# csiro-robotics/ohm

Hardware: AMD Instinct MI355X
Metric: rays/sec integrated (occupancy) (higher is better)
Workload: dtype f64

## Files before the change

### include/ohmhip.h

```cpp
#ifndef OHMHIP_H
#define OHMHIP_H

#include <stddef.h>
#include <stdint.h>

#ifdef __cplusplus
extern "C" {
#endif

#define OHMHIP_EXPERIMENTAL

#define OHMHIP_OK 0
#define OHMHIP_ERR_INVALID_ARG (-1)
#define OHMHIP_ERR_NO_DEVICE (-2)
#define OHMHIP_ERR_CAPACITY (-3)
#define OHMHIP_ERR_UNSUPPORTED (-4)
#define OHMHIP_ERR_NOT_FOUND (-5)
#define OHMHIP_ERR_INTERNAL (-6)
#define OHMHIP_ERR_PEER (-7)

const char *ohmhip_error_string(int status);
const char *ohmhip_build_id(void);

typedef struct ohmhip_stream_s *ohmhip_stream_t;
// ... 152 lines not shown
                                     const float *d_intensities, const double *d_timestamps, unsigned ray_flags,
                                     size_t *integrated);
typedef struct ohmhip_cache_stats
{
  uint64_t hits;
  uint64_t misses;
  uint64_t full;
  uint32_t regions_resident;
  uint32_t region_capacity;
  uint64_t bytes_per_region;
  uint64_t memory_limit;
  uint64_t evictions;
  uint64_t readmissions;
  uint32_t regions_spilled;
  uint32_t spill_enabled;
  uint64_t writebacks;
  uint64_t writeback_hits;
  uint64_t writeback_stale;
} ohmhip_cache_stats;
int ohmhip_map_cache_stats(ohmhip_map_t map, ohmhip_cache_stats *stats, int reset);
int ohmhip_map_set_memory_limit(ohmhip_map_t map, uint64_t bytes);
int ohmhip_map_set_spill_to_host(ohmhip_map_t map, int enable);
OHMHIP_EXPERIMENTAL int ohmhip_map_set_spill_writeback(ohmhip_map_t map, int enable);
int ohmhip_map_sync(ohmhip_map_t map);
int ohmhip_map_last_stats(ohmhip_map_t map, ohmhip_batch_stats *stats);

OHMHIP_EXPERIMENTAL int ohmhip_map_batch_timings(ohmhip_map_t map, uint32_t batches_back, float ms[4]);
OHMHIP_EXPERIMENTAL int ohmhip_map_set_phase_timing(ohmhip_map_t map, int enable);
OHMHIP_EXPERIMENTAL int ohmhip_map_reserve_rays(ohmhip_map_t map, size_t ray_count);
int ohmhip_map_set_first_ray_time(ohmhip_map_t map, double time);
int ohmhip_map_first_ray_time(ohmhip_map_t map, double *time);
OHMHIP_EXPERIMENTAL int ohmhip_map_batches_launched(ohmhip_map_t map, uint64_t *count);
OHMHIP_EXPERIMENTAL int ohmhip_map_pipeline_counts(ohmhip_map_t map, uint64_t *batches, uint64_t *binned_early);
OHMHIP_EXPERIMENTAL int ohmhip_map_rays_beyond_tiles(ohmhip_map_t map, uint64_t *count);

int ohmhip_map_region_count(ohmhip_map_t map, size_t *count);
int ohmhip_map_regions(ohmhip_map_t map, int16_t *keys_xyz, size_t capacity, size_t *count);
int ohmhip_map_dirty_regions(ohmhip_map_t map, int16_t *keys_xyz, size_t capacity, size_t *count);
int ohmhip_map_clear_dirty(ohmhip_map_t map);
size_t ohmhip_layer_voxel_bytes(int layer_id);

int ohmhip_map_read_regions(ohmhip_map_t map, int layer_id, const int16_t *keys_xyz, size_t count, void *const *dsts);
int ohmhip_map_write_regions(ohmhip_map_t map, int layer_id, const int16_t *keys_xyz, size_t count,
                             const void *const *srcs);
int ohmhip_map_clear(ohmhip_map_t map);
int ohmhip_map_remove_regions(ohmhip_map_t map, const int16_t *keys_xyz, size_t count, size_t *removed);

int ohmhip_map_line_keys(ohmhip_map_t map, const double *lines, size_t line_count, uint32_t max_keys_per_line,
                         void *keys_out, uint32_t *counts_out);

int ohmhip_map_rays_query(ohmhip_map_t map, const double *rays, size_t element_count, double volume_coefficient,
                          double *ranges, double *unobserved_volumes, int8_t *terminal_types, void *terminal_keys);
OHMHIP_EXPERIMENTAL int ohmhip_map_rays_query_device(ohmhip_map_t map, const double *d_rays, size_t element_count,
                                                     double volume_coefficient, double *d_ranges,
                                                     double *d_unobserved_volumes, int8_t *d_terminal_types,
                                                     void *d_terminal_keys);

#define OHMHIP_QF_UNKNOWN_AS_OCCUPIED (1u << 0)
#define OHMHIP_QF_REPORT_UNSCALED (1u << 4)
typedef struct ohmhip_clearance_params
{
  float search_radius;
  float axis_scaling[3];
  unsigned flags;
} ohmhip_clearance_params;

// ... 264 lines not shown
```

### ohm_amd/_lib.py

```python
import ctypes as C
import os

_HERE = os.path.dirname(os.path.abspath(__file__))
LIB_PATH = os.environ.get("OHMHIP_LIB") or os.path.join(_HERE, "lib", "libohmhip.so")


class OhmHipError(RuntimeError):
    def __init__(self, status, what=""):
        self.status = status
        msg = lib.ohmhip_error_string(status).decode() if "lib" in globals() else str(status)
        super().__init__(f"{what}: [{status}] {msg}" if what else f"[{status}] {msg}")


if not os.path.exists(LIB_PATH):
    raise ImportError(
        f"{LIB_PATH} is missing: build it with `python -c 'import __graft_entry__ as g; g.build()'` "
        "(hipcc --offload-arch=gfx950). ohm_amd has no CPU fallback.")

lib = C.CDLL(LIB_PATH)

OK = 0
ERR_INVALID_ARG, ERR_NO_DEVICE, ERR_CAPACITY, ERR_UNSUPPORTED, ERR_NOT_FOUND, ERR_INTERNAL, ERR_PEER = (-1, -2, -3, -4,
                                                                                                       -5, -6, -7)
MERGE_SHARED_ONLY, MERGE_FULL_UNION = 0, 1
# ... 172 lines not shown
    "ohmhip_map_sync": (C.c_int, [_vp]),
    "ohmhip_map_last_stats": (C.c_int, [_vp, C.POINTER(BatchStats)]),
    "ohmhip_map_region_count": (C.c_int, [_vp, C.POINTER(C.c_size_t)]),
    "ohmhip_map_regions": (C.c_int, [_vp, _vp, C.c_size_t, C.POINTER(C.c_size_t)]),
    "ohmhip_map_dirty_regions": (C.c_int, [_vp, _vp, C.c_size_t, C.POINTER(C.c_size_t)]),
    "ohmhip_map_clear_dirty": (C.c_int, [_vp]),
    "ohmhip_map_read_regions": (C.c_int, [_vp, C.c_int, _vp, C.c_size_t, _vp]),
    "ohmhip_map_write_regions": (C.c_int, [_vp, C.c_int, _vp, C.c_size_t, _vp]),
    "ohmhip_map_clear": (C.c_int, [_vp]),
    "ohmhip_map_remove_regions": (C.c_int, [_vp, _vp, C.c_size_t, C.POINTER(C.c_size_t)]),
    "ohmhip_transform_samples": (C.c_int, [_vp, _vp, _vp, C.c_uint32, _vp, _vp, C.c_uint32, C.c_double, _vp, _vp,
                                           C.POINTER(C.c_uint32)]),
    "ohmhip_pattern_create": (C.c_int, [_vp, C.c_size_t, C.POINTER(_vp)]),
    "ohmhip_pattern_destroy": (C.c_int, [_vp]),
    "ohmhip_pattern_ray_count": (C.c_int, [_vp, C.POINTER(C.c_size_t)]),
    "ohmhip_pattern_build_rays": (C.c_int, [_vp, _vp, C.c_size_t, C.c_int, C.c_double, _vp]),
    "ohmhip_pattern_last_rays": (C.c_int, [_vp, _vp, C.POINTER(C.c_size_t)]),
    "ohmhip_map_apply_pattern": (C.c_int, [_vp, _vp, _vp, C.c_size_t, C.c_int, C.c_double, C.c_float, C.c_uint,
                                           C.POINTER(C.c_size_t)]),
    "ohmhip_map_can_copy": (C.c_int, [_vp, _vp]),
    "ohmhip_map_copy": (C.c_int, [_vp, _vp, C.POINTER(CopyParams), C.POINTER(CopyStats)]),
    "ohmhip_map_compare": (C.c_int, [_vp, _vp, C.POINTER(CompareParams), C.c_uint64, _vp, C.c_uint64, _vp,
                                     C.POINTER(CompareResult)]),
    "ohmhip_map_compare_device": (C.c_int, [_vp, _vp, C.POINTER(CompareParams), C.c_uint64, _vp, C.c_uint64, _vp, _vp]),
    "ohmhip_map_batch_timings": (C.c_int, [_vp, C.c_uint32, C.POINTER(C.c_float)]),
    "ohmhip_comm_exchange_side": (C.c_int, [_vp, _vp, _vp, _vp, _vp, C.c_uint32, _vp]),
    "ohmhip_gather_rows": (C.c_int, [_vp, _vp, C.c_size_t, C.c_uint32, _vp, _vp]),
    "ohmhip_map_reserve_rays": (C.c_int, [_vp, C.c_size_t]),
    "ohmhip_map_set_first_ray_time": (C.c_int, [_vp, C.c_double]),
    "ohmhip_map_first_ray_time": (C.c_int, [_vp, C.POINTER(C.c_double)]),
    "ohmhip_map_set_phase_timing": (C.c_int, [_vp, C.c_int]),
    "ohmhip_map_batches_launched": (C.c_int, [_vp, C.POINTER(C.c_uint64)]),
    "ohmhip_map_pipeline_counts": (C.c_int, [_vp, C.POINTER(C.c_uint64), C.POINTER(C.c_uint64)]),
    "ohmhip_map_rays_beyond_tiles": (C.c_int, [_vp, C.POINTER(C.c_uint64)]),
    "ohmhip_map_line_keys": (C.c_int, [_vp, _vp, C.c_size_t, C.c_uint32, _vp, _vp]),
    "ohmhip_map_rays_query": (C.c_int, [_vp, _vp, C.c_size_t, C.c_double, _vp, _vp, _vp, _vp]),
    "ohmhip_map_rays_query_device": (C.c_int, [_vp, _vp, C.c_size_t, C.c_double, _vp, _vp, _vp, _vp]),
    "ohmhip_map_clearance_regions": (C.c_int, [_vp, _vp, C.c_size_t, _vp, _vp]),
    "ohmhip_map_clearance_regions_device": (C.c_int, [_vp, _vp, C.c_size_t, _vp, _vp]),
    "ohmhip_map_clearance_keys": (C.c_int, [_vp, _vp, C.c_size_t, _vp, _vp]),
    "ohmhip_map_clearance_stale_regions": (C.c_int, [_vp, _vp, _vp, C.c_size_t, C.POINTER(C.c_size_t)]),
    "ohmhip_map_clearance_update": (C.c_int, [_vp, _vp, C.c_size_t, C.POINTER(C.c_size_t), C.POINTER(C.c_size_t)]),
    "ohmhip_map_clearance_update_regions": (C.c_int, [_vp, _vp, C.c_size_t, _vp, C.c_int, C.POINTER(C.c_size_t)]),
    "ohmhip_map_heightmap_extents": (C.c_int, [_vp, C.POINTER(HeightmapParams), C.POINTER(HeightmapExtents)]),
    "ohmhip_map_heightmap": (C.c_int, [_vp, C.POINTER(HeightmapParams), _vp, _vp, _vp, _vp, C.POINTER(C.c_uint64),
                                       C.POINTER(C.c_uint64)]),
    "ohmhip_map_heightmap_device": (C.c_int, [_vp, C.POINTER(HeightmapParams), _vp, _vp, _vp, _vp, _vp]),
    "ohmhip_map_heightmap_fill_extents": (C.c_int, [_vp, C.POINTER(HeightmapParams), C.POINTER(HeightmapExtents)]),
    "ohmhip_map_heightmap_fill": (C.c_int, [_vp, C.POINTER(HeightmapParams), _vp, _vp, _vp, _vp, _vp, C.c_uint64,
                                            C.POINTER(HeightmapFillStats)]),
    "ohmhip_map_heightmap_fill_device": (C.c_int, [_vp, C.POINTER(HeightmapParams), _vp, _vp, _vp, _vp, _vp, C.c_uint64,
                                                   C.POINTER(HeightmapFillStats)]),
    "ohmhip_map_cloud_count": (C.c_int, [_vp, C.POINTER(CloudParams), C.POINTER(C.c_uint64)]),
    "ohmhip_map_cloud": (C.c_int, [_vp, C.POINTER(CloudParams), C.c_uint64, _vp, _vp, _vp, C.POINTER(C.c_uint64)]),
    "ohmhip_map_cloud_device": (C.c_int, [_vp, C.POINTER(CloudParams), C.c_uint64, _vp, _vp, _vp, _vp]),
    "ohmhip_map_nearest_neighbours": (C.c_int, [_vp, _vp, C.c_size_t, C.POINTER(NeighboursParams), C.c_uint64, _vp, _vp,
                                                _vp, C.POINTER(C.c_uint64)]),
    "ohmhip_map_nearest_neighbours_device": (C.c_int, [_vp, _vp, C.c_size_t, C.POINTER(NeighboursParams), C.c_uint64,
                                                       _vp, _vp, _vp, _vp]),
    "ohmhip_map_voxel_keys": (C.c_int, [_vp, _vp, C.c_size_t, _vp]),
    "ohmhip_map_read_voxels": (C.c_int, [_vp, C.c_int, _vp, C.c_size_t, _vp, _vp]),
    "ohmhip_map_read_voxels_device": (C.c_int, [_vp, C.c_int, _vp, C.c_size_t, _vp, _vp]),
    "ohmhip_map_filter_points": (C.c_int, [_vp, _vp, C.c_uint64, C.POINTER(PointFilterParams), C.c_uint64, _vp, _vp, _vp,
                                           _vp, C.POINTER(C.c_uint64)]),
    "ohmhip_map_filter_points_device": (C.c_int, [_vp, _vp, C.c_uint64, C.c_uint64, C.POINTER(PointFilterParams),
                                                  C.c_uint64, _vp, _vp, _vp, _vp, _vp]),
# ... 46 lines not shown
```

### ohm_amd/csrc/batch_run.h

```cpp
#ifndef OHMHIP_BATCH_RUN_H
#define OHMHIP_BATCH_RUN_H

namespace
{
struct BatchRun
{
  ohmhip_map_t m;
  const double *d_rays;
  const float *d_intensities;
  const double *d_timestamps;
  uint32_t n_rays;
  unsigned ray_flags;
  hipStream_t s, f;
  const Event *tev;
  uint32_t ring;
  uint32_t next_info_index = 0;
  bool info_clean = false;
  uint32_t ray_blocks = 0, bin_rays_per_block = 0, bin_threads = 0, bin_blocks = 0, bin_tab_mask = 0;
  uint32_t batch_chunk_segments = 0;
  int mode = 0;
  bool stop_mode = false, occupancy_mode = false, ndt_mode = false, tsdf_mode = false;
  bool occ_inline = false;
  int ray_shift = 0;
  SecondaryLayers sec;
// ... 73 lines not shown
    }
    if (occupancy_mode)
    {
      OHMHIP_CHECK(m->hit_keys_a.ensure(sizeof(unsigned long long) * size_t(n_rays), false, s));
      OHMHIP_CHECK(m->hit_keys_b.ensure(sizeof(unsigned long long) * size_t(n_rays), false, s));
      OHMHIP_CHECK(m->interval_counts.ensure(sizeof(uint32_t) * size_t(n_rays), true, s));
      size_t sort_bytes = 0;
      OHMHIP_CHECK(rocprim::radix_sort_keys<SortConfig>(nullptr, sort_bytes, static_cast<unsigned long long *>(m->hit_keys_a.ptr),
                                            static_cast<unsigned long long *>(m->hit_keys_b.ptr), size_t(n_rays),
                                            kHitRayBits, sortEndBit(m), s));
      OHMHIP_CHECK(m->sort_temp.ensure(sort_bytes, false, s));
    }
    return OHMHIP_OK;
  }

  uint32_t *binMask() const { return occupancy_mode ? nullptr : m->pool.d_hit_mask.get(); }

  void launchBin(bool bucket, uint32_t seg_capacity, unsigned long long *hit_keys, hipStream_t stream)
  {
    const auto pow2 = [](int v) { return (v & (v - 1)) == 0; };
    const bool plain = m->mc.owner_world <= 1u && pow2(m->mc.dim[0]) && pow2(m->mc.dim[1]) && pow2(m->mc.dim[2]);
    const bool small = bin_tab_mask < kLtabSmall;
    const auto kernel = small ? (plain ? k_ray_bin<kLtabSmall, true> : k_ray_bin<kLtabSmall, false>) :
                                (plain ? k_ray_bin<kLtabSize, true> : k_ray_bin<kLtabSize, false>);
    hipExtLaunchKernelGGL(kernel, dim3(bin_blocks), dim3(bin_threads), 0, stream, nullptr, tev[1], 0, m->mc,
                          regionTable(m), batchScratch(m), static_cast<const RayWalk *>(batchWalks(m).ptr), n_rays,
                          static_cast<Segment *>(m->segments.ptr), seg_capacity, hit_keys, binMask(), ray_shift,
                          bucket ? 1 : 0, bin_rays_per_block, bin_tab_mask);
    mark(1);
    m->tev_pre_walk[ring] = 1;
    m->bin_done_event = tev[1];
  }

  void launchRegionSort(uint32_t dense)
  {
    const unsigned long long *in = static_cast<const unsigned long long *>(m->hit_keys_a.ptr);
    unsigned long long *out = static_cast<unsigned long long *>(m->hit_keys_b.ptr);
    const bool need_dense = kSortSmallHits == 0 || dense > kSortSmallHits;
    if (need_dense)
    {
      hipExtLaunchKernelGGL((k_sort_region_hits<kSortRegionHits, kSortThreads>), dim3(2 * m->walk_workgroups),
                            dim3(kSortThreads), 0, s, nullptr, kSortSmallHits ? nullptr : tev[2].handle, 0, regionTable(m),
                            batchScratch(m), in, out, m->mc.region_voxels, kSortSmallHits, m->pool.d_hit_mask.get());
    }
    if (kSortSmallHits)
    {
      hipExtLaunchKernelGGL((k_sort_region_hits<kSortSmallHits ? kSortSmallHits : 64u, kSortSmallThreads>),
                            dim3(8 * m->walk_workgroups), dim3(kSortSmallThreads), 0, s, nullptr, tev[2], 0,
                            regionTable(m), batchScratch(m), in, out, m->mc.region_voxels, 0u, m->pool.d_hit_mask.get());
    }
    sort_covers = need_dense ? kSortRegionHits : kSortSmallHits;
    mark(2);
    m->tev_pre_walk[ring] = 2;
  }

  void launchDenseSort()
  {
    hipExtLaunchKernelGGL((k_sort_region_hits<kSortRegionHits, kSortThreads>), dim3(2 * m->walk_workgroups),
                          dim3(kSortThreads), 0, s, nullptr, tev[2], 0, regionTable(m), batchScratch(m),
                          static_cast<const unsigned long long *>(m->hit_keys_a.ptr),
                          static_cast<unsigned long long *>(m->hit_keys_b.ptr), m->mc.region_voxels, kSortSmallHits,
                          m->pool.d_hit_mask.get());
    sort_covers = kSortRegionHits;
  }

  int frontHalf()
  {
    if (m->batch_done_event[m->parity])
    {
      OHMHIP_CHECK(hipStreamWaitEvent(f, m->batch_done_event[m->parity], 0));
    }
    if (m->bin_done_event)
    {
      OHMHIP_CHECK(hipStreamWaitEvent(f, m->bin_done_event, 0));
    }
    if (attempt > 0 || !info_clean)
    {
      OHMHIP_CHECK(hipMemsetAsync(m->d_info + m->info_index, 0, sizeof(BatchInfo), f));
    }
    if (m->phase_timing)
    {
      OHMHIP_CHECK(hipEventRecord(tev[0], f));
      mark(0);
    }
    if (bin_tab_mask < kLtabSmall)
    {
      hipLaunchKernelGGL(k_ray_setup<kLtabSmall>, dim3(bin_blocks), dim3(bin_threads), 0, f, m->mc, regionTable(m),
                         batchScratch(m), d_rays, n_rays, ray_flags, static_cast<RayWalk *>(batchWalks(m).ptr),
                         bin_rays_per_block, bin_tab_mask);
    }
    else
    {
      hipLaunchKernelGGL(k_ray_setup<kLtabSize>, dim3(bin_blocks), dim3(bin_threads), 0, f, m->mc, regionTable(m),
                         batchScratch(m), d_rays, n_rays, ray_flags, static_cast<RayWalk *>(batchWalks(m).ptr),
                         bin_rays_per_block, bin_tab_mask);
// ... 623 lines not shown
```

### ohm_amd/csrc/map_state.h

```cpp
#ifndef OHMHIP_MAP_STATE_H
#define OHMHIP_MAP_STATE_H

namespace
{
const size_t kLayerBytes[OHMHIP_LID_COUNT] = { 4, 8, 24, 4, 4, 4, 8, 8, 8, 4 };

inline uint32_t layerClearWord(int l)
{
  return (l == OHMHIP_LID_OCCUPANCY) ? 0x7f800000u : (l == OHMHIP_LID_CLEARANCE) ? 0xbf800000u : 0u;
}


struct DevBuf
{
  void *ptr = nullptr;
  size_t bytes = 0;

  DevBuf() = default;
  DevBuf(DevBuf &&o) noexcept : ptr(o.ptr), bytes(o.bytes) { o.ptr = nullptr, o.bytes = 0; }
  DevBuf &operator=(DevBuf &&o) noexcept
  {
    if (this != &o)
    {
      release();
// ... 314 lines not shown
    DevBuf clear_regions, clear_keys, clear_out, clear_mask;
    DevBuf hm_winner, hm_rec_occ, hm_rec_vox, hm_rec_mean, hm_counts, hm_out_occ, hm_out_vox, hm_out_mean, hm_out_col;
    DevBuf hmf_grid, hmf_queue, hmf_ground, hmf_rec_cell, hmf_keys_a, hmf_keys_b, hmf_accept, hmf_accept_at, hmf_temp, hmf_log;
    PinnedBuf<uint32_t> hmf_next;
    DevBuf cloud_chunks, cloud_pos, cloud_keys, cloud_values;
    ScanScratch cloud_scan;
    DevBuf nn_chunks, nn_chunk_begin, nn_near, nn_best, nn_query_counts, nn_query_best, nn_keys, nn_ranges;
    ScanScratch nn_scan, nn_query_scan;
    DevBuf rv_keys, rv_values, rv_present;
    DevBuf pf_points, pf_status, pf_values, pf_keys, pf_kept;
    ScanScratch pf_scan;
    PinnedBuf<char> pf_staging;
    DevBuf compare_chunks, compare_records, compare_keys, compare_missing, compare_result;
    ScanScratch compare_scan;
  } query;
  struct ClearanceLayerState
  {
    struct Region
    {
      uint32_t changed = 0;
      uint32_t written = 0;
      uint32_t params = 0;
    };
    std::unordered_map<uint64_t, Region> regions;
    uint32_t epoch = 0;
    std::vector<ohmhip_clearance_params> param_sets;
    DevBuf table_keys, table_changed, present, written, stale;
  } clearance_layer;
  DevArray<uint32_t> d_event_count;
  uint32_t walk_workgroups = 256;
  bool walk_half = false;
  uint32_t walkSlots() const { return walk_workgroups * (walk_half ? 2u : 1u); }
  DevArray<unsigned long long> d_dbg;
  double first_ray_time = -1.0;
  uint32_t event_demand = 0;
  uint32_t event_limit = 0;
  bool spec_bucket_ok = false;
  uint32_t spec_max_region_hits = 0;
  double segments_per_ray = 10.0;
  uint32_t bin_rays_per_block = kBinRaysPerBlock;
  uint32_t min_chunk_segments = 2048;
  uint32_t chunk_segments = kChunkSegments;
  unsigned debug_flags = 0;
  int refill_min_idle = kRefillMinIdle;
  PinnedBuf<void> h_stage;
  size_t h_stage_bytes = 0;

  struct RaySlot
  {
    PinnedBuf<char> h;
    size_t capacity = 0;
    DevBuf d_rays, d_times, d_intens, d_fflags;
    Event uploaded;
    Event done;
    bool in_flight = false;
    bool rays_uploaded = false;
  } ray_slots[2];
  std::unique_ptr<StagePool> stage_pool;
  bool async_launch = false;
  std::unique_ptr<StagePool> launch_thread;
  bool launch_busy = false;
  int launch_result = OHMHIP_OK;
  int fill_slot = 0;
  size_t pending_rays = 0;
  size_t pending_calls = 0;
  unsigned pending_flags = 0;
// ... 124 lines not shown
```

### ohm_amd/csrc/ohmhip_map.hip

```cpp
#include <cstring>
#include <string.h>

#include "apply_kernels.h"
#include "batch_scratch.h"
#include "pool_kernels.h"
#include "ray_front_kernels.h"
#include "region_table.h"
#include "sample_sort_kernels.h"
#include "walk_kernel.h"
#include "replay_kernels.h"
#include "traversal_kernels.h"
#include "query_kernels.h"
#include "clearance_kernels.h"
#include "heightmap_kernels.h"
#include "heightmap_fill_kernels.h"
#include "cloud_kernels.h"
#include "neighbours_kernels.h"
#include "point_filter_kernels.h"
#include "copy_kernels.h"
#include "compare_kernels.h"

#include <rocprim/rocprim.hpp>

#include <algorithm>
// ... 139 lines not shown
    mc.fix_scale = double(kFixMaxDelta) / (1.01 * diagonal);
    mc.fix_margin = 2u * uint32_t(std::max(mc.dim[0], std::max(mc.dim[1], mc.dim[2]))) + 8u;
  }
  applyValueConfig(m);

  if (hipGetDevice(&m->device) != hipSuccess)
  {
    return OHMHIP_ERR_NO_DEVICE;
  }
  OHMHIP_CHECK(m->stream.create());
  OHMHIP_CHECK(m->copy_stream.create());
  OHMHIP_CHECK(m->front_stream.create());
  for (auto &e : m->ev)
  {
    OHMHIP_CHECK(e.create());
  }
  for (auto &set : m->tev)
  {
    for (auto &e : set)
    {
      OHMHIP_CHECK(e.create());
    }
  }
  for (auto &sl : m->ray_slots)
  {
    OHMHIP_CHECK(sl.uploaded.create(hipEventDisableTiming));
    OHMHIP_CHECK(sl.done.create(hipEventDisableTiming));
  }
  OHMHIP_CHECK(m->d_n_slots.alloc(sizeof(uint32_t)));
  OHMHIP_CHECK(m->d_info.alloc(3 * sizeof(BatchInfo)));
  OHMHIP_CHECK(m->d_event_count.alloc(8 * sizeof(uint32_t)));
  OHMHIP_CHECK(m->d_dbg.alloc(kDbgWords * sizeof(unsigned long long)));
  (void)hipMemset(m->d_dbg, 0, kDbgWords * sizeof(unsigned long long));
  OHMHIP_CHECK(m->h_info.alloc(2 * sizeof(BatchInfo), hipHostMallocMapped | hipHostMallocCoherent));
  std::memset(m->h_info, 0, 2 * sizeof(BatchInfo));
  OHMHIP_CHECK(m->h_passed.alloc(64, hipHostMallocMapped | hipHostMallocCoherent));
  OHMHIP_CHECK(m->ev_passed.create(hipEventDisableTiming));

  uint32_t capacity = m->config.region_capacity;
  if (capacity == 0)
  {
    const uint64_t budget = m->config.gpu_mem_size ? m->config.gpu_mem_size : (uint64_t(4) << 30);
    capacity = uint32_t(std::max<uint64_t>(64, budget / bytesPerRegionAllLayers(m->config, mc.region_voxels)));
  }
  capacity = std::min<uint32_t>(capacity, kMaxRegionSlots);
  OHMHIP_CHECK(allocPool(m, capacity, 0));
  {
    int device = 0, cus = 0;
    if (hipGetDevice(&device) == hipSuccess &&
        hipDeviceGetAttribute(&cus, hipDeviceAttributeMultiprocessorCount, device) == hipSuccess && cus > 0)
    {
      m->walk_workgroups = uint32_t(cus);
    }
  }
  if (const char *env = std::getenv("OHMHIP_CHUNK_SEGMENTS"))
  {
    m->chunk_segments = uint32_t(std::max(64, std::min(int(kMaxChunkSegments), std::atoi(env))));
  }
  if (const char *env = std::getenv("OHMHIP_EVENT_LIMIT"))
  {
    m->event_limit = uint32_t(std::max(0, std::atoi(env)));
  }
  if (const char *env = std::getenv("OHMHIP_WRITEBACK"))
  {
    m->writeback_off = std::atoi(env) == 0;
  }
  if (const char *env = std::getenv("OHMHIP_WRITEBACK_WGS"))
  {
    m->writeback_workgroups = uint32_t(std::max(1, std::min(4096, std::atoi(env))));
  }
  if (const char *env = std::getenv("OHMHIP_BIN_RAYS"))
  {
    m->bin_rays_per_block = uint32_t(std::max(128, std::min(int(kBinRaysPerBlock), std::atoi(env))));
  }
  if (const char *env = std::getenv("OHMHIP_MIN_CHUNK_SEGMENTS"))
  {
    m->min_chunk_segments = uint32_t(std::max(64, std::min(int(kMaxChunkSegments), std::atoi(env))));
  }
  if (const char *env = std::getenv("OHMHIP_EARLY_BIN"))
  {
    m->early_bin = std::atoi(env) != 0;
  }
  uint32_t half_voxels = uint32_t(WalkHalf::kTileVoxels) / 4u;
  if (const char *env = std::getenv("OHMHIP_WALK_HALF_VOXELS"))
  {
    half_voxels = uint32_t(std::max(0, std::min(int(WalkHalf::kTileVoxels), std::atoi(env))));
// ... 435 lines not shown
int ohmhip_map_batches_launched(ohmhip_map_t m, uint64_t *count)
try
{
  if (!m || !count)
  {
    return OHMHIP_ERR_INVALID_ARG;
  }
  if (m->launch_busy)
  {
    m->launch_thread->wait();
  }
  *count = m->batch_seq;
  return OHMHIP_OK;
}
OHMHIP_ABI_CATCH

int ohmhip_map_pipeline_counts(ohmhip_map_t m, uint64_t *batches, uint64_t *binned_early)
try
{
  if (!m || !batches || !binned_early)
  {
    return OHMHIP_ERR_INVALID_ARG;
  }
  if (m->launch_busy)
  {
    m->launch_thread->wait();
  }
  *batches = m->count_batches;
  *binned_early = m->count_binned_early;
  return OHMHIP_OK;
}
OHMHIP_ABI_CATCH

int ohmhip_map_cache_stats(ohmhip_map_t m, ohmhip_cache_stats *stats, int reset)
try
{
  if (!m || !stats)
  {
    return OHMHIP_ERR_INVALID_ARG;
  }
  OHMHIP_SETTLE(m);
  stats->hits = m->cache_hits;
  stats->misses = m->cache_misses;
  stats->full = m->cache_full;
  stats->regions_resident = m->slots_committed;
  stats->region_capacity = m->pool.slot_capacity;
  stats->bytes_per_region = bytesPerRegionAllLayers(m->config, m->mc.region_voxels);
  stats->memory_limit = m->memory_limit;
  stats->evictions = m->evictions;
  stats->readmissions = m->readmissions;
  stats->regions_spilled = uint32_t(m->spilled.size());
  stats->spill_enabled = m->spill_enabled ? 1u : 0u;
  stats->writebacks = m->writebacks;
  stats->writeback_hits = m->writeback_hits;
  stats->writeback_stale = m->writeback_stale;
  if (reset)
  {
    m->cache_hits = m->cache_misses = m->cache_full = 0;
    m->evictions = m->readmissions = 0;
    m->writebacks = m->writeback_hits = m->writeback_stale = 0;
  }
  return OHMHIP_OK;
}
OHMHIP_ABI_CATCH

int ohmhip_map_set_memory_limit(ohmhip_map_t m, uint64_t bytes)
// ... 198 lines not shown
```

### ohm_amd/csrc/sample_sort_kernels.h

```cpp
#ifndef OHMHIP_SAMPLE_SORT_KERNELS_H
#define OHMHIP_SAMPLE_SORT_KERNELS_H

#include "batch_scratch.h"
#include "region_table.h"

namespace ohmhip
{
__global__ void __launch_bounds__(256)
  k_hit_bounds(const unsigned long long *__restrict__ sorted, BatchScratch bs, int region_voxels,
               uint32_t *__restrict__ hit_mask)
{
  const uint32_t n_hits = bs.info->n_hits;
  const uint32_t i = blockIdx.x * blockDim.x + threadIdx.x;
  if (i >= n_hits)
  {
    return;
  }
  const unsigned long long group = hitGroup(sorted[i]);
  if (i == 0 || hitGroup(sorted[i - 1]) != group)
  {
    const uint32_t slot = hitSlot(sorted[i]);
    const uint32_t vi = hitVoxel(sorted[i]);
    bs.voxel_first_hit[size_t(slot) * size_t(region_voxels) + vi] = i;
    atomicOr(&hit_mask[size_t(slot) * (uint32_t(region_voxels + 31) >> 5) + (vi >> 5)], 1u << (vi & 31));
// ... 21 lines not shown
  const uint32_t low = g & ((1u << s_shift) - 1u);
  const uint32_t base = ((g >> s_shift) << (s_shift + R)) | low;
  const bool ascending = (base & k) == 0;
  unsigned long long v[kCount];
#pragma unroll
  for (uint32_t m = 0; m < kCount; ++m)
  {
    v[m] = l_keys[sortSlot(base | (m << s_shift))];
  }
#pragma unroll
  for (int t = 0; t < R; ++t)
  {
    const uint32_t d = 1u << (R - 1 - t);
#pragma unroll
    for (uint32_t m = 0; m < kCount; ++m)
    {
      if ((m & d) == 0)
      {
        const unsigned long long a = v[m];
        const unsigned long long c = v[m | d];
        const bool swap = (a > c) == ascending;
        v[m] = swap ? c : a;
        v[m | d] = swap ? a : c;
      }
    }
  }
#pragma unroll
  for (uint32_t m = 0; m < kCount; ++m)
  {
    l_keys[sortSlot(base | (m << s_shift))] = v[m];
  }
}

constexpr uint32_t kSortRegionHits = 8192;
constexpr int kSortThreads = 1024;
#ifndef OHMHIP_SORT_SMALL
#define OHMHIP_SORT_SMALL 2048
#endif
constexpr uint32_t kSortSmallHits = OHMHIP_SORT_SMALL;
constexpr int kSortSmallThreads = 256;

template <uint32_t kCap, int kThreads>
__global__ void __launch_bounds__(kThreads)
  k_sort_region_hits(RegionTable rt, BatchScratch bs, const unsigned long long *__restrict__ keys,
                     unsigned long long *__restrict__ sorted, int region_voxels, uint32_t min_hits,
                     uint32_t *__restrict__ hit_mask)
{
  __shared__ unsigned long long l_keys[kCap + kCap / 32];
  const uint32_t mask_words = uint32_t(region_voxels + 31) >> 5;
  const uint32_t n_regions = bs.info->n_hit_regions;
  for (uint32_t list_index = blockIdx.x; list_index < n_regions; list_index += gridDim.x)
  {
  const uint32_t h = bs.sort_list[list_index];
  const uint32_t slot = rt.vals[h];
  if (slot >= rt.slot_capacity)
  {
    continue;
  }
  const uint32_t begin = bs.hit_begin[slot];
  const uint32_t n = bs.hit_end[slot] - begin;
  if (n <= min_hits || n > kCap)
  {
    continue;
  }
  uint32_t padded = 64;
  while (padded < n)
  {
    padded <<= 1;
  }
  for (uint32_t i = threadIdx.x; i < padded; i += kThreads)
  {
    l_keys[sortSlot(i)] = (i < n) ? keys[begin + i] : ~0ull;
  }
  __syncthreads();
  for (uint32_t k = 2; k <= padded; k <<= 1)
  {
    uint32_t j = k >> 1;
    while (j > 0)
    {
      const uint32_t levels_left = uint32_t(32 - __clz(int(j)));
      const uint32_t r = min(3u, levels_left);
      const uint32_t s_shift = levels_left - r;
      const uint32_t group_count = padded >> r;
      for (uint32_t g = threadIdx.x; g < group_count; g += kThreads)
      {
        if (r == 3)
        {
          bitonicFused<3>(l_keys, g, s_shift, k);
        }
        else if (r == 2)
        {
          bitonicFused<2>(l_keys, g, s_shift, k);
        }
        else
        {
          bitonicFused<1>(l_keys, g, s_shift, k);
        }
      }
      __syncthreads();
      j >>= r;
    }
  }
  for (uint32_t base = 0; base < n; base += kThreads)
  {
    const uint32_t i = base + threadIdx.x;
    uint32_t word = 0xffffffffu, bits = 0;
    if (i < n)
    {
      const unsigned long long key = l_keys[sortSlot(i)];
      sorted[begin + i] = key;
      const uint32_t vi = hitVoxel(key);
      word = vi >> 5;
      if (i == 0 || hitGroup(l_keys[sortSlot(i - 1)]) != hitGroup(key))
      {
        bs.voxel_first_hit[size_t(slot) * size_t(region_voxels) + vi] = begin + i;
        bits = 1u << (vi & 31);
      }
    }
    const uint32_t lane = threadIdx.x & 63u;
#pragma unroll
    for (uint32_t d = 1; d < 64u; d <<= 1)
    {
      const uint32_t up_bits = __shfl_up(bits, d, 64);
      const uint32_t up_word = __shfl_up(word, d, 64);
      bits |= (lane >= d && up_word == word) ? up_bits : 0u;
    }
    const uint32_t next_word = __shfl_down(word, 1u, 64);
    if (bits && (lane == 63u || next_word != word))
    {
      atomicOr(&hit_mask[size_t(slot) * mask_words + word], bits);
    }
  }
  __syncthreads();
  }
}

__global__ void k_stream_marker() {}

__global__ void __launch_bounds__(256) k_reset_cursors(RegionTable rt, BatchScratch bs)
{
  const uint32_t i = blockIdx.x * blockDim.x + threadIdx.x;
  if (i >= bs.info->n_touched)
  {
    return;
  }
  const uint32_t h = bs.touched[i];
  bs.seg_cursor[h] = 0;
  const uint32_t slot = rt.vals[h];
  if (slot < rt.slot_capacity)
  {
    bs.hit_end[slot] = bs.hit_begin[slot];
  }
}
}

#endif
```

### ohm_amd/gpumap.py

```python
import ctypes as C
import enum
import math
import time

import numpy as np

from . import _lib as L


class RayFlag(enum.IntFlag):
    kRfDefault = 0
    kRfEndPointAsFree = 1 << 0
    kRfStopOnFirstOccupied = 1 << 1
    kRfExcludeOrigin = 1 << 2
    kRfExcludeSample = 1 << 3
    kRfExcludeRay = 1 << 4
    kRfExcludeUnobserved = 1 << 5
    kRfExcludeFree = 1 << 6
    kRfExcludeOccupied = 1 << 7
    kRfReverseWalk = 1 << 8


class OccupancyType(enum.IntEnum):
    kNull = -2
# ... 331 lines not shown

    def stats(self):
        st = L.BatchStats()
        L.check(L.lib.ohmhip_map_last_stats(self._handle, C.byref(st)), "stats")
        return {name: getattr(st, name) for name, _ in L.BatchStats._fields_}

    def batchTimings(self, batches_back=0):
        ms = (C.c_float * 4)()
        L.check(L.lib.ohmhip_map_batch_timings(self._handle, batches_back, ms), "batch_timings")
        return {"ms_total": ms[0], "ms_setup": ms[1], "ms_walk": ms[2], "ms_apply": ms[3]}

    def setFirstRayTime(self, time):
        L.check(L.lib.ohmhip_map_set_first_ray_time(self._handle, float(time)), "set_first_ray_time")
        self._time_base_checked = False

    def firstRayTime(self):
        t = C.c_double(-1.0)
        L.check(L.lib.ohmhip_map_first_ray_time(self._handle, C.byref(t)), "first_ray_time")
        return float(t.value)

    def setPhaseTiming(self, enable=True):
        L.check(L.lib.ohmhip_map_set_phase_timing(self._handle, 1 if enable else 0), "set_phase_timing")

    def batchesLaunched(self):
        n = C.c_uint64(0)
        L.check(L.lib.ohmhip_map_batches_launched(self._handle, C.byref(n)), "batches_launched")
        return int(n.value)

    def pipelineCounts(self):
        batches, early = C.c_uint64(0), C.c_uint64(0)
        L.check(L.lib.ohmhip_map_pipeline_counts(self._handle, C.byref(batches), C.byref(early)), "pipeline_counts")
        return int(batches.value), int(early.value)

    def raysBeyondTiles(self):
        n = C.c_uint64(0)
        L.check(L.lib.ohmhip_map_rays_beyond_tiles(self._handle, C.byref(n)), "rays_beyond_tiles")
        return int(n.value)

    def wait(self):
        L.check(L.lib.ohmhip_map_sync(self._handle), "sync")

    def gpuCache(self):
        owner = self

        class _GpuCacheView:
            def flush(self):
                owner.syncVoxels()

            def clear(self):
                owner.clear()

            def remove(self, region_key):
                owner.removeRegions([region_key])

            def reinitialise(self):
                owner.clear()

            def targetGpuAllocSize(self):
                return int(owner.cacheStats()["memory_limit"])

            def layerCount(self):
                return len(owner.map().layers)

        return _GpuCacheView()

    def removeRegions(self, keys):
# ... 895 lines not shown
```

Baseline: 1.202 billion.

## Sort region hits by voxel-bucket counting and rank, falling back to bitonic

Replaces the per-region bitonic sort of hit keys with a counting pass over voxel buckets, a prefix scan, a scatter into bucket ranges, and a small in-bucket rank computation. A sum of squared bucket sizes decides per region whether this is cheap enough; otherwise the bitonic network still runs. This aims to cut the log-squared compare-exchange passes and barriers of the bitonic sort for regions whose hits are spread across many voxels. It adds extra shared memory, extra key reads from global memory, a launch bound hint, an optional sort grid cap via an environment variable, and device counters with an API to read them.

```diff
diff --git a/include/ohmhip.h b/include/ohmhip.h
--- a/include/ohmhip.h
+++ b/include/ohmhip.h
@@ -208,6 +208,7 @@
 int ohmhip_map_first_ray_time(ohmhip_map_t map, double *time);
 OHMHIP_EXPERIMENTAL int ohmhip_map_batches_launched(ohmhip_map_t map, uint64_t *count);
 OHMHIP_EXPERIMENTAL int ohmhip_map_pipeline_counts(ohmhip_map_t map, uint64_t *batches, uint64_t *binned_early);
+OHMHIP_EXPERIMENTAL int ohmhip_map_order_counts(ohmhip_map_t map, uint64_t *regions_ranked, uint64_t *regions_network);
 OHMHIP_EXPERIMENTAL int ohmhip_map_rays_beyond_tiles(ohmhip_map_t map, uint64_t *count);
 
 int ohmhip_map_region_count(ohmhip_map_t map, size_t *count);
diff --git a/ohm_amd/_lib.py b/ohm_amd/_lib.py
--- a/ohm_amd/_lib.py
+++ b/ohm_amd/_lib.py
@@ -228,6 +228,7 @@
     "ohmhip_map_set_phase_timing": (C.c_int, [_vp, C.c_int]),
     "ohmhip_map_batches_launched": (C.c_int, [_vp, C.POINTER(C.c_uint64)]),
     "ohmhip_map_pipeline_counts": (C.c_int, [_vp, C.POINTER(C.c_uint64), C.POINTER(C.c_uint64)]),
+    "ohmhip_map_order_counts": (C.c_int, [_vp, C.POINTER(C.c_uint64), C.POINTER(C.c_uint64)]),
     "ohmhip_map_rays_beyond_tiles": (C.c_int, [_vp, C.POINTER(C.c_uint64)]),
     "ohmhip_map_line_keys": (C.c_int, [_vp, _vp, C.c_size_t, C.c_uint32, _vp, _vp]),
     "ohmhip_map_rays_query": (C.c_int, [_vp, _vp, C.c_size_t, C.c_double, _vp, _vp, _vp, _vp]),
diff --git a/ohm_amd/csrc/batch_run.h b/ohm_amd/csrc/batch_run.h
--- a/ohm_amd/csrc/batch_run.h
+++ b/ohm_amd/csrc/batch_run.h
@@ -129,6 +129,12 @@
     m->bin_done_event = tev[1];
   }
 
+  uint32_t sortGrid(uint32_t per_cu) const
+  {
+    const uint32_t grid = per_cu * m->walk_workgroups;
+    return m->sort_workgroups ? std::min(grid, m->sort_workgroups) : grid;
+  }
+
   void launchRegionSort(uint32_t dense)
   {
     const unsigned long long *in = static_cast<const unsigned long long *>(m->hit_keys_a.ptr);
@@ -136,15 +142,17 @@
     const bool need_dense = kSortSmallHits == 0 || dense > kSortSmallHits;
     if (need_dense)
     {
-      hipExtLaunchKernelGGL((k_sort_region_hits<kSortRegionHits, kSortThreads>), dim3(2 * m->walk_workgroups),
+      hipExtLaunchKernelGGL((k_sort_region_hits<kSortRegionHits, kSortThreads>), dim3(sortGrid(2)),
                             dim3(kSortThreads), 0, s, nullptr, kSortSmallHits ? nullptr : tev[2].handle, 0, regionTable(m),
-                            batchScratch(m), in, out, m->mc.region_voxels, kSortSmallHits, m->pool.d_hit_mask.get());
+                            batchScratch(m), in, out, m->mc.region_voxels, kSortSmallHits, m->pool.d_hit_mask.get(),
+                            m->d_order_counts.get());
     }
     if (kSortSmallHits)
     {
       hipExtLaunchKernelGGL((k_sort_region_hits<kSortSmallHits ? kSortSmallHits : 64u, kSortSmallThreads>),
-                            dim3(8 * m->walk_workgroups), dim3(kSortSmallThreads), 0, s, nullptr, tev[2], 0,
-                            regionTable(m), batchScratch(m), in, out, m->mc.region_voxels, 0u, m->pool.d_hit_mask.get());
+                            dim3(sortGrid(8)), dim3(kSortSmallThreads), 0, s, nullptr, tev[2], 0,
+                            regionTable(m), batchScratch(m), in, out, m->mc.region_voxels, 0u, m->pool.d_hit_mask.get(),
+                            m->d_order_counts.get());
     }
     sort_covers = need_dense ? kSortRegionHits : kSortSmallHits;
     mark(2);
@@ -153,11 +161,11 @@
 
   void launchDenseSort()
   {
-    hipExtLaunchKernelGGL((k_sort_region_hits<kSortRegionHits, kSortThreads>), dim3(2 * m->walk_workgroups),
+    hipExtLaunchKernelGGL((k_sort_region_hits<kSortRegionHits, kSortThreads>), dim3(sortGrid(2)),
                           dim3(kSortThreads), 0, s, nullptr, tev[2], 0, regionTable(m), batchScratch(m),
                           static_cast<const unsigned long long *>(m->hit_keys_a.ptr),
                           static_cast<unsigned long long *>(m->hit_keys_b.ptr), m->mc.region_voxels, kSortSmallHits,
-                          m->pool.d_hit_mask.get());
+                          m->pool.d_hit_mask.get(), m->d_order_counts.get());
     sort_covers = kSortRegionHits;
   }
 
diff --git a/ohm_amd/csrc/map_state.h b/ohm_amd/csrc/map_state.h
--- a/ohm_amd/csrc/map_state.h
+++ b/ohm_amd/csrc/map_state.h
@@ -370,6 +370,8 @@
   bool walk_half = false;
   uint32_t walkSlots() const { return walk_workgroups * (walk_half ? 2u : 1u); }
   DevArray<unsigned long long> d_dbg;
+  DevArray<unsigned long long> d_order_counts;
+  uint32_t sort_workgroups = 0;
   double first_ray_time = -1.0;
   uint32_t event_demand = 0;
   uint32_t event_limit = 0;
diff --git a/ohm_amd/csrc/ohmhip_map.hip b/ohm_amd/csrc/ohmhip_map.hip
--- a/ohm_amd/csrc/ohmhip_map.hip
+++ b/ohm_amd/csrc/ohmhip_map.hip
@@ -195,6 +195,8 @@
   OHMHIP_CHECK(m->d_event_count.alloc(8 * sizeof(uint32_t)));
   OHMHIP_CHECK(m->d_dbg.alloc(kDbgWords * sizeof(unsigned long long)));
   (void)hipMemset(m->d_dbg, 0, kDbgWords * sizeof(unsigned long long));
+  OHMHIP_CHECK(m->d_order_counts.alloc(2 * sizeof(unsigned long long)));
+  OHMHIP_CHECK(hipMemset(m->d_order_counts, 0, 2 * sizeof(unsigned long long)));
   OHMHIP_CHECK(m->h_info.alloc(2 * sizeof(BatchInfo), hipHostMallocMapped | hipHostMallocCoherent));
   std::memset(m->h_info, 0, 2 * sizeof(BatchInfo));
   OHMHIP_CHECK(m->h_passed.alloc(64, hipHostMallocMapped | hipHostMallocCoherent));
@@ -215,6 +217,10 @@
     {
       m->walk_workgroups = uint32_t(cus);
     }
+  }
+  if (const char *env = std::getenv("OHMHIP_SORT_WORKGROUPS"))
+  {
+    m->sort_workgroups = uint32_t(std::max(0, std::atoi(env)));
   }
   if (const char *env = std::getenv("OHMHIP_CHUNK_SEGMENTS"))
   {
@@ -716,6 +722,26 @@
 }
 OHMHIP_ABI_CATCH
 
+int ohmhip_map_order_counts(ohmhip_map_t m, uint64_t *regions_ranked, uint64_t *regions_network)
+try
+{
+  if (!m || !regions_ranked || !regions_network)
+  {
+    return OHMHIP_ERR_INVALID_ARG;
+  }
+  if (m->launch_busy)
+  {
+    m->launch_thread->wait();
+  }
+  OHMHIP_CHECK(hipStreamSynchronize(m->stream));
+  unsigned long long counts[2] = { 0, 0 };
+  OHMHIP_CHECK(hipMemcpy(counts, m->d_order_counts, sizeof(counts), hipMemcpyDeviceToHost));
+  *regions_ranked = counts[0];
+  *regions_network = counts[1];
+  return OHMHIP_OK;
+}
+OHMHIP_ABI_CATCH
+
 int ohmhip_map_cache_stats(ohmhip_map_t m, ohmhip_cache_stats *stats, int reset)
 try
 {
diff --git a/ohm_amd/csrc/sample_sort_kernels.h b/ohm_amd/csrc/sample_sort_kernels.h
--- a/ohm_amd/csrc/sample_sort_kernels.h
+++ b/ohm_amd/csrc/sample_sort_kernels.h
@@ -77,47 +77,9 @@
   }
 }
 
-constexpr uint32_t kSortRegionHits = 8192;
-constexpr int kSortThreads = 1024;
-#ifndef OHMHIP_SORT_SMALL
-#define OHMHIP_SORT_SMALL 2048
-#endif
-constexpr uint32_t kSortSmallHits = OHMHIP_SORT_SMALL;
-constexpr int kSortSmallThreads = 256;
-
-template <uint32_t kCap, int kThreads>
-__global__ void __launch_bounds__(kThreads)
-  k_sort_region_hits(RegionTable rt, BatchScratch bs, const unsigned long long *__restrict__ keys,
-                     unsigned long long *__restrict__ sorted, int region_voxels, uint32_t min_hits,
-                     uint32_t *__restrict__ hit_mask)
-{
-  __shared__ unsigned long long l_keys[kCap + kCap / 32];
-  const uint32_t mask_words = uint32_t(region_voxels + 31) >> 5;
-  const uint32_t n_regions = bs.info->n_hit_regions;
-  for (uint32_t list_index = blockIdx.x; list_index < n_regions; list_index += gridDim.x)
-  {
-  const uint32_t h = bs.sort_list[list_index];
-  const uint32_t slot = rt.vals[h];
-  if (slot >= rt.slot_capacity)
-  {
-    continue;
-  }
-  const uint32_t begin = bs.hit_begin[slot];
-  const uint32_t n = bs.hit_end[slot] - begin;
-  if (n <= min_hits || n > kCap)
-  {
-    continue;
-  }
-  uint32_t padded = 64;
-  while (padded < n)
-  {
-    padded <<= 1;
-  }
-  for (uint32_t i = threadIdx.x; i < padded; i += kThreads)
-  {
-    l_keys[sortSlot(i)] = (i < n) ? keys[begin + i] : ~0ull;
-  }
-  __syncthreads();
+template <int kThreads>
+__device__ inline void bitonicNetwork(unsigned long long *l_keys, uint32_t padded, uint32_t tid)
+{
   for (uint32_t k = 2; k <= padded; k <<= 1)
   {
     uint32_t j = k >> 1;
@@ -127,7 +89,7 @@
       const uint32_t r = min(3u, levels_left);
       const uint32_t s_shift = levels_left - r;
       const uint32_t group_count = padded >> r;
-      for (uint32_t g = threadIdx.x; g < group_count; g += kThreads)
+      for (uint32_t g = tid; g < group_count; g += kThreads)
       {
         if (r == 3)
         {
@@ -146,9 +108,196 @@
       j >>= r;
     }
   }
+}
+
+constexpr uint32_t kSortRegionHits = 8192;
+constexpr int kSortThreads = 1024;
+#ifndef OHMHIP_SORT_SMALL
+#define OHMHIP_SORT_SMALL 2048
+#endif
+constexpr uint32_t kSortSmallHits = OHMHIP_SORT_SMALL;
+constexpr int kSortSmallThreads = 256;
+
+#ifndef OHMHIP_ORDER_SHIFT_SMALL
+#define OHMHIP_ORDER_SHIFT_SMALL 5
+#endif
+#ifndef OHMHIP_ORDER_SHIFT_DENSE
+#define OHMHIP_ORDER_SHIFT_DENSE 5
+#endif
+#ifndef OHMHIP_ORDER_RANK_LIMIT
+#define OHMHIP_ORDER_RANK_LIMIT 32
+#endif
+constexpr uint32_t kOrderRankLimit = OHMHIP_ORDER_RANK_LIMIT;
+static_assert(kSortRegionHits < 65536u, "bucket positions are 16-bit halves");
+constexpr unsigned long long kBelowSlot = (1ull << kHitSlotShift) - 1ull;
+static_assert(kSortRegionHits <= (1u << (64 - kHitSlotShift)), "a key's final position travels in its slot field");
+
+template <uint32_t kCap, int kThreads>
+__global__ void __launch_bounds__(kThreads, 8)
+  k_sort_region_hits(RegionTable rt, BatchScratch bs, const unsigned long long *__restrict__ keys,
+                     unsigned long long *__restrict__ sorted, int region_voxels, uint32_t min_hits,
+                     uint32_t *__restrict__ hit_mask, unsigned long long *__restrict__ order_counts)
+{
+  constexpr uint32_t kPerLane = (kCap + uint32_t(kThreads) - 1u) / uint32_t(kThreads);
+  constexpr uint32_t kWaves = uint32_t(kThreads) / 64u;
+  constexpr uint32_t kOrderShift = kThreads == kSortThreads ? OHMHIP_ORDER_SHIFT_DENSE : OHMHIP_ORDER_SHIFT_SMALL;
+  constexpr uint32_t kOrderWords = ((1u << kHitVoxelBits) >> kOrderShift) / 2u;
+  constexpr uint32_t kScanLanes = uint32_t(kThreads) < kOrderWords ? uint32_t(kThreads) : kOrderWords;
+  constexpr uint32_t kScanWords = kOrderWords / kScanLanes;
+  static_assert(kThreads % 64 == 0 && kCap <= kSortRegionHits, "launch shape");
+  __shared__ unsigned long long l_keys[kCap + kCap / 32];
+  __shared__ uint32_t l_bucket[kOrderWords];
+  __shared__ uint32_t l_wave_sum[kWaves], l_wave_sq[kWaves];
+  const uint32_t mask_words = uint32_t(region_voxels + 31) >> 5;
+  const uint32_t n_regions = bs.info->n_hit_regions;
+  for (uint32_t list_index = blockIdx.x; list_index < n_regions; list_index += gridDim.x)
+  {
+  const uint32_t h = bs.sort_list[list_index];
+  const uint32_t slot = rt.vals[h];
+  if (slot >= rt.slot_capacity)
+  {
+    continue;
+  }
+  const uint32_t begin = bs.hit_begin[slot];
+  const uint32_t n = bs.hit_end[slot] - begin;
+  if (n <= min_hits || n > kCap)
+  {
+    continue;
+  }
+  uint32_t tid = threadIdx.x;
+  asm volatile("" : "+v"(tid));
+  const uint32_t lane = tid & 63u;
+  const uint32_t wave = tid >> 6;
+  for (uint32_t w = tid; w < kOrderWords; w += kThreads)
+  {
+    l_bucket[w] = 0;
+  }
+  __syncthreads();
+#pragma unroll 2
+  for (uint32_t i = tid; i < n; i += kThreads)
+  {
+    const unsigned long long key = keys[begin + i];
+    l_keys[sortSlot(i)] = key;
+    const uint32_t b = hitVoxel(key) >> kOrderShift;
+    atomicAdd(&l_bucket[b >> 1], 1u << ((b & 1u) * 16u));
+  }
+  __syncthreads();
+  uint32_t sum = 0, sq = 0;
+#pragma unroll
+  for (uint32_t w = 0; w < kScanWords; ++w)
+  {
+    const uint32_t word = tid < kScanLanes ? l_bucket[tid * kScanWords + w] : 0u;
+    sum += (word & 0xffffu) + (word >> 16);
+    sq += (word & 0xffffu) * (word & 0xffffu) + (word >> 16) * (word >> 16);
+  }
+  uint32_t inclusive = sum;
+#pragma unroll
+  for (uint32_t d = 1; d < 64u; d <<= 1)
+  {
+    const uint32_t up = __shfl_up(inclusive, d, 64);
+    inclusive += lane >= d ? up : 0u;
+    sq += __shfl_xor(sq, d, 64);
+  }
+  if (lane == 63u)
+  {
+    l_wave_sum[wave] = inclusive;
+    l_wave_sq[wave] = sq;
+  }
+  __syncthreads();
+  uint32_t position = inclusive - sum, compares = 0;
+#pragma unroll
+  for (uint32_t w = 0; w < kWaves; ++w)
+  {
+    position += w < wave ? l_wave_sum[w] : 0u;
+    compares += l_wave_sq[w];
+  }
+  const bool ranked = kOrderRankLimit != 0 &&
+                      __builtin_amdgcn_readfirstlane(compares) <= kOrderRankLimit * n;
+  if (ranked)
+  {
+    if (tid < kScanLanes)
+    {
+#pragma unroll
+      for (uint32_t w = 0; w < kScanWords; ++w)
+      {
+        const uint32_t word = l_bucket[tid * kScanWords + w];
+        const uint32_t first = position;
+        position += word & 0xffffu;
+        l_bucket[tid * kScanWords + w] = first | (position << 16);
+        position += word >> 16;
+      }
+    }
+    __syncthreads();
+#pragma unroll 2
+    for (uint32_t i = tid; i < n; i += kThreads)
+    {
+      const unsigned long long key = keys[begin + i];
+      const uint32_t b = hitVoxel(key) >> kOrderShift;
+      const uint32_t half = (b & 1u) * 16u;
+      const uint32_t place = (atomicAdd(&l_bucket[b >> 1], 1u << half) >> half) & 0xffffu;
+      l_keys[sortSlot(place)] = key & kBelowSlot;
+    }
+    __syncthreads();
+#pragma unroll 1
+    for (uint32_t i = tid; i < n; i += kThreads)
+    {
+      const unsigned long long key = l_keys[sortSlot(i)];
+      const uint32_t b = hitVoxel(key) >> kOrderShift;
+      const uint32_t range_end = (l_bucket[b >> 1] >> ((b & 1u) * 16u)) & 0xffffu;
+      const uint32_t range_begin = b ? (l_bucket[(b - 1u) >> 1] >> (((b - 1u) & 1u) * 16u)) & 0xffffu : 0u;
+      uint32_t rank = 0;
+#pragma unroll 4
+      for (uint32_t q = range_begin; q < range_end; ++q)
+      {
+        const unsigned long long other = l_keys[sortSlot(q)] & kBelowSlot;
+        rank += (other < key || (other == key && q < i)) ? 1u : 0u;
+      }
+      l_keys[sortSlot(i)] = key | ((unsigned long long)(range_begin + rank) << kHitSlotShift);
+    }
+    __syncthreads();
+    unsigned long long own[kPerLane];
+#pragma unroll
+    for (uint32_t j = 0; j < kPerLane; ++j)
+    {
+      const uint32_t i = j * kThreads + tid;
+      own[j] = i < n ? l_keys[sortSlot(i)] : 0ull;
+    }
+    __syncthreads();
+#pragma unroll
+    for (uint32_t j = 0; j < kPerLane; ++j)
+    {
+      if (j * kThreads + tid < n)
+      {
+        l_keys[sortSlot(uint32_t(own[j] >> kHitSlotShift))] =
+          (own[j] & kBelowSlot) | ((unsigned long long)slot << kHitSlotShift);
+      }
+    }
+    __syncthreads();
+  }
+  else
+  {
+    uint32_t padded = 64;
+    while (padded < n)
+    {
+      padded <<= 1;
+    }
+    for (uint32_t i = n + tid; i < padded; i += kThreads)
+    {
+      l_keys[sortSlot(i)] = kHitInvalid;
+    }
+    __syncthreads();
+    bitonicNetwork<kThreads>(l_keys, padded, tid);
+  }
+  if (threadIdx.x == 0 && order_counts)
+  {
+    atomicAdd(&order_counts[ranked ? 0 : 1], 1ull);
+  }
+  uint32_t tail_tid = threadIdx.x;
+  asm volatile("" : "+v"(tail_tid));
+  const uint32_t tail_lane = tail_tid & 63u;
   for (uint32_t base = 0; base < n; base += kThreads)
   {
-    const uint32_t i = base + threadIdx.x;
+    const uint32_t i = base + tail_tid;
     uint32_t word = 0xffffffffu, bits = 0;
     if (i < n)
     {
@@ -162,16 +311,15 @@
         bits = 1u << (vi & 31);
       }
     }
-    const uint32_t lane = threadIdx.x & 63u;
 #pragma unroll
     for (uint32_t d = 1; d < 64u; d <<= 1)
     {
       const uint32_t up_bits = __shfl_up(bits, d, 64);
       const uint32_t up_word = __shfl_up(word, d, 64);
-      bits |= (lane >= d && up_word == word) ? up_bits : 0u;
+      bits |= (tail_lane >= d && up_word == word) ? up_bits : 0u;
     }
     const uint32_t next_word = __shfl_down(word, 1u, 64);
-    if (bits && (lane == 63u || next_word != word))
+    if (bits && (tail_lane == 63u || next_word != word))
     {
       atomicOr(&hit_mask[size_t(slot) * mask_words + word], bits);
     }
diff --git a/ohm_amd/gpumap.py b/ohm_amd/gpumap.py
--- a/ohm_amd/gpumap.py
+++ b/ohm_amd/gpumap.py
@@ -387,6 +387,11 @@
         L.check(L.lib.ohmhip_map_pipeline_counts(self._handle, C.byref(batches), C.byref(early)), "pipeline_counts")
         return int(batches.value), int(early.value)
 
+    def orderCounts(self):
+        ranked, network = C.c_uint64(0), C.c_uint64(0)
+        L.check(L.lib.ohmhip_map_order_counts(self._handle, C.byref(ranked), C.byref(network)), "order_counts")
+        return int(ranked.value), int(network.value)
+
     def raysBeyondTiles(self):
         n = C.c_uint64(0)
         L.check(L.lib.ohmhip_map_rays_beyond_tiles(self._handle, C.byref(n)), "rays_beyond_tiles")
```

After: 1.222 billion, median of 6. +1.7%, better.
